# 21K1113/Neural_Image_Compression_V2

Measured on AMD Instinct MI355X. Metric: Mpixels/sec train-step (fwd+bwd) + PSNR, 4K RGB, 1/2/4/8 MI355X, higher is better.
Workload: dtype bf16x2-split operands, f32 accumulate

## Files before the change

neural_image_compression_v2_amd/csrc/fused_train16.hpp:

```cpp
#pragma once
#include "fused_kernel.hpp"


#ifndef NIC_T16_HALF16
#define NIC_T16_HALF16 1
#endif
#ifndef NIC_T16_LOFF
#define NIC_T16_LOFF 26
#endif
#ifndef NIC_T16_PIN
#define NIC_T16_PIN 0
#endif
namespace nic {

struct Lds16 {
    static constexpr int LD1 = 80, LD2 = 80, LD3 = 80;
    static constexpr int LDZ = 72, LDX = 88;
    static constexpr int KP = 80;
    static constexpr int OFF_W1 = 0;
    static constexpr int W1LO = kH * LD1;
    static constexpr int OFF_W2 = OFF_W1 + 2 * kH * LD1;
    static constexpr int W2LO = kH * LD2;
    static constexpr int OFF_W3 = OFF_W2 + 2 * kH * LD2;
    static constexpr int W3LO = 4 * LD3;
    static constexpr int OFF_B = OFF_W3 + 2 * 4 * LD3;
    static constexpr int OFF_IMG = OFF_B + 144;
    static constexpr int DZLO = 16 * LDZ, OFF_A1 = 2 * 16 * LDZ, OFF_X = 4 * 16 * LDZ, XLO = 16 * LDX, OFF_D3 = OFF_X + 2 * 16 * LDX;
    static constexpr int SPW = OFF_D3 + 128;
    static constexpr int TOTAL = OFF_IMG + 8 * SPW;
    static_assert(TOTAL * 2 <= 163840, "LDS");
    static_assert(OFF_IMG % 8 == 0 && SPW % 8 == 0 && OFF_B % 8 == 0, "16-byte alignment");
    static constexpr int REC_W2 = 0, REC_W1 = 8 * 1024, REC_TAIL = 16 * 1024, REC_WAVE = REC_TAIL + 8 * 256, REC = REC_WAVE + 8 * 320;
};

__host__ __device__ constexpr int slot16_channel(int s, int g) {
    if (s < 12) return 12 * g + s;
    if (s < 15) return 48 + 3 * g + (s - 12);
    if (s == 15) return kSlotZero;
    if (s < 19) return 60 + 3 * g + (s - 16);
    if (s == 19) return g == 0 ? 72 : (g == 1 ? kSlotOne : kSlotZero);
    return kSlotZero;
}
__host__ __device__ constexpr int channel_of_rho16(int rho) {
    if (rho < 64) return slot16_channel(8 * (rho >> 5) + (rho & 7), (rho >> 3) & 3);
    return slot16_channel(16 + (rho & 3), (rho - 64) >> 2);
}
__host__ __device__ constexpr int rho16_of_channel(int ch) {
    for (int rho = 0; rho < Lds16::KP; ++rho)
        if (channel_of_rho16(rho) == ch) return rho;
    return -1;
}
__host__ __device__ constexpr int pos16(int h) { return 32 * (h >> 5) + 8 * ((h >> 2) & 3) + 4 * ((h >> 4) & 1) + (h & 3); }
__host__ __device__ constexpr int hid16(int pos) { return 16 * (2 * (pos >> 5) + ((pos >> 2) & 1)) + 4 * ((pos >> 3) & 3) + (pos & 3); }

typedef __attribute__((address_space(3))) const u32x4 lds_cu4;
typedef __attribute__((address_space(3))) u32x4 lds_u4;
__device__ __forceinline__ bf16x8 ld_frag(lds_cbf* p) { return __builtin_bit_cast(bf16x8, *reinterpret_cast<lds_cu4*>(p)); }
__device__ __forceinline__ void st_frag(lds_bf* p, const bf16x8& f) { *reinterpret_cast<lds_u4*>(p) = __builtin_bit_cast(u32x4, f); }
__device__ __forceinline__ bf16x8 half_frag(s16x4 a) {
    const s16x8 v = {a[0], a[1], a[2], a[3], 0, 0, 0, 0};
    return __builtin_bit_cast(bf16x8, v);
}
struct Half2 {
    s16x4 hi, lo;
};
__device__ __forceinline__ f32x4 mfma16h_bf(s16x4 a, s16x4 b, f32x4 c) { return __builtin_amdgcn_mfma_f32_16x16x16bf16_1k(a, b, c, 0, 0, 0); }
__device__ __forceinline__ f32x4 mfma16h_split(const Half2& a, const Half2& b, f32x4 c) {
    c = mfma16h_bf(a.lo, b.hi, c);
    c = mfma16h_bf(a.hi, b.lo, c);
    return mfma16h_bf(a.hi, b.hi, c);
}
__device__ __forceinline__ f32x4 mfma16_split(const Frag2& a, const Frag2& b, f32x4 c) {
    c = mfma16_bf(a.lo, b.hi, c);
    c = mfma16_bf(a.hi, b.lo, c);
    return mfma16_bf(a.hi, b.hi, c);
}
__device__ __forceinline__ Frag2 split_pair(const f32x4& a, const f32x4& b) {
    const float x[8] = {a[0], a[1], a[2], a[3], b[0], b[1], b[2], b[3]};
    return split8(x);
}
__device__ __forceinline__ lds_bf* opaque(lds_bf* p) {
#ifndef NIC_NO_OPAQUE_PTR
    asm volatile("" : "+v"(p));
#endif
    return p;
}

#ifndef NIC_T16_PF
#define NIC_T16_PF 2
#endif
template <int NT, bool ZERO = false, class LoadA>
__device__ __forceinline__ void kstep16(f32x4 (&acc)[NT], const Frag2& bf, LoadA&& load_a) {
    constexpr int PF = NIC_T16_PF < NT ? NIC_T16_PF : NT;
    Frag2 af[PF];
#pragma unroll
    for (int t = 0; t < PF; ++t) af[t] = load_a(t);
#pragma unroll
    for (int t = 0; t < NT; ++t) {
        acc[t] = mfma16_split(af[t % PF], bf, ZERO ? f32x4(0.f) : acc[t]);
        if (t + PF < NT) af[t % PF] = load_a(t + PF);
    }
}

struct CellRaw16 {
    float g0[kC];
    float g1[4 * 3];
};
struct GridAcc16 {
    float g1[4 * 3];
};

__device__ __forceinline__ int opaque_i(int v) {
#ifndef NIC_NO_OPAQUE_LANE
    asm volatile("" : "+v"(v));
#endif
    return v;
}

__device__ __forceinline__ float grid_load16(const char* base, uint32_t ob, int kind, const FusedParams& p) {
    if (kind == 0) return *reinterpret_cast<const float*>(base + ob);
    if (kind == 3) {
        const float n = (float)*reinterpret_cast<const uint8_t*>(base + ob) - p.dq_sub;
        const float q = mul_rn(n, p.dq_rcp);
        return fmaf(fmaf(-q, p.dq_den, n), p.dq_rcp, q);
    }
    const uint32_t hbits = *reinterpret_cast<const uint16_t*>(base + ob);
    if (kind == 1) return __builtin_bit_cast(float, hbits << 16);
    return (float)__builtin_bit_cast(_Float16, (uint16_t)hbits);
}
__device__ __forceinline__ void gather_cell16_kind(const FusedParams& p, const int kind, uint32_t off0, uint32_t off1, int g, CellRaw16& raw) {
    const uint32_t eb = kind == 0 ? 4u : (kind == 3 ? 1u : 2u);
    const uint32_t pb0 = (uint32_t)p.g0.plane * eb, pb1 = (uint32_t)p.g1.plane * eb;
    {
        uint32_t ob = (off0 + (uint32_t)p.g0.at(g >> 1, g & 1, 0)) * eb;
        const char* base = reinterpret_cast<const char*>(p.g0.p);
#pragma unroll
        for (int c = 0; c < kC; ++c, ob += pb0) raw.g0[c] = grid_load16(base, ob, kind, p);
    }
#pragma unroll
    for (int c4 = 0; c4 < 4; ++c4) {
        uint32_t ob = (off1 + (uint32_t)p.g1.at(c4 >> 1, c4 & 1, 0)) * eb + (uint32_t)(3 * g) * pb1;
        const char* base = reinterpret_cast<const char*>(p.g1.p);
#pragma unroll
        for (int cc = 0; cc < 3; ++cc, ob += pb1) raw.g1[c4 * 3 + cc] = grid_load16(base, ob, kind, p);
    }
}
__device__ __forceinline__ void gather_cell16(const FusedParams& p, uint32_t off0, uint32_t off1, int g, CellRaw16& raw) {
    gather_cell16_kind(p, p.grid_kind, off0, off1, g, raw);
}
__device__ __forceinline__ void gather_cell16_switched(const FusedParams& p, uint32_t off0, uint32_t off1, int g, CellRaw16& raw) {
    switch (p.grid_kind) {
        case 0: gather_cell16_kind(p, 0, off0, off1, g, raw); break;
        case 1: gather_cell16_kind(p, 1, off0, off1, g, raw); break;
        case 3: gather_cell16_kind(p, 3, off0, off1, g, raw); break;
        default: gather_cell16_kind(p, 2, off0, off1, g, raw); break;
    }
}

template <class L>
__device__ __forceinline__ void encode16(const FusedParams& p, const int (&q)[3], int g, float (&xs)[20], EncCtx& cx, const CellRaw16& raw) {
    const nic_path_desc& d = p.d;
    const int e = d.log2_step;
    const Axis ax = axis_coords(q[0], e), ay = axis_coords(q[1], e);
    cx.kx = ax.k1; cx.ky = ay.k1; cx.kz = 0.f;
#pragma unroll
    for (int c = 0; c < kC; ++c) xs[c] = raw.g0[c];
    {
        const float c = (g >> 1) ? ay.t1 : ax.t1;
#pragma unroll
        for (int i = 0; i < 3; ++i) {
            const int r = 3 * (g & 1) + i;
            float v;
            if (L::PE == NIC_PE_TRIANGULAR) {
                v = tri_pe_row(c, r, kP);
            } else {
                const int k = r >> 1;
                const float dv = k == 0 ? d.pe_div[0] : (k == 1 ? d.pe_div[1] : d.pe_div[2]);
                float sv, cv;
                sincos_cw(mul_rn(c, dv), sv, cv);
                v = (r & 1) ? cv : sv;
            }
            xs[15 + i] = v;
        }
        xs[18] = g == 0 ? d.lod_value : (g == 1 ? 1.0f : 0.f);
    }
    const G1FactorsT<2> gf = g1_factors<2>(d.g1_weight_mode, cx.kx, cx.ky, 0.f);
#pragma unroll
    for (int cc = 0; cc < 3; ++cc) {
        float sum = 0.f;
#pragma unroll
        for (int c4 = 0; c4 < 4; ++c4) {
            const uint32_t b = (gf.bits >> (3 * c4)) & 7u;
            float v = raw.g1[c4 * 3 + cc];
            v = mul_rn(v, (b & 1u) ? gf.fx[1] : gf.fx[0]);
            v = mul_rn(v, (b & 2u) ? gf.fy[1] : gf.fy[0]);
            sum = c4 == 0 ? v : add_rn(sum, v);
        }
        xs[12 + cc] = sum;
    }
}
__host__ __device__ constexpr int xs_of_slot(int s) { return s < 15 ? s : s - 1; }

template <class L>
__device__ __forceinline__ void add_noise16(const NoiseSrc& ns, uint64_t sample_global, int64_t n_local, int g, float (&xs)[20]) {
    if (ns.mode == NIC_NOISE_NONE) return;
    if (ns.mode == NIC_NOISE_TENSOR) {
        const float* row = ns.tensor + n_local * L::CIN;
#pragma unroll
        for (int s = 0; s < 20; ++s) {
            if (s == 15) continue;
            const int ch0 = slot16_channel(s, 0);
            if (s == 19) { xs[18] += g == 0 ? row[72] : 0.f; continue; }
            const int stride = slot16_channel(s, 1) - ch0;
            xs[xs_of_slot(s)] += row[ch0 + stride * g];
        }
        return;
    }
    const U4 b = noise_block(ns, sample_global, g);
#pragma unroll
    for (int f = 0; f < 18; ++f) xs[f] += noise_field(ns, b, f);
    const float nl = noise_field(ns, b, 18);
    xs[18] += g == 0 ? nl : 0.f;
}

__device__ __forceinline__ int shfl_lane(int v, int src_lane) { return __builtin_amdgcn_ds_bpermute(src_lane << 2, v); }
__device__ __forceinline__ float shfl_lane(float v, int src_lane) { return __builtin_bit_cast(float, __builtin_amdgcn_ds_bpermute(src_lane << 2, __builtin_bit_cast(int, v))); }
__device__ __forceinline__ void combine_g1_lanes16(GridAcc16& ga, uint32_t off1, const int (&blk)[3], int lane, int lw) {
    const int T[2] = {1 << lw, 16 >> lw};
    const int STR[2] = {1, 1 << lw};
    const int pl = lane & 15;
    const int lc[2] = {pl & (T[0] - 1), pl >> lw};
#pragma unroll
    for (int a = 0; a < 2; ++a) {
        const bool odd = blk[a] & 1;
        const int pc = lc[a] + (odd ? -1 : 1);
        const bool inb = pc >= 0 && pc < T[a];
        const int partner = inb ? lane + (odd ? -STR[a] : STR[a]) : lane;
        const bool pair = inb && (uint32_t)shfl_lane((int)off1, partner) == off1;
#pragma unroll
        for (int i = 0; i < 12; ++i) {
            const float pv = shfl_lane(ga.g1[i], partner);
            ga.g1[i] = pair ? (odd ? 0.f : ga.g1[i] + pv) : ga.g1[i];
        }
    }
}

__device__ __forceinline__ void preadd_x16(f32x4 (&dxacc)[4], uint32_t off0, int ln) {
    const int n16 = ln & 15, g = ln >> 4;
    const bool recv = g < 2;
    const bool inb = recv ? n16 >= 1 : n16 <= 14;
    const int partner = inb ? (recv ? ln + 31 : ln - 31) : ln;
    const uint32_t poff = (uint32_t)shfl_lane((int)off0, partner);
    const bool pair = inb && (recv ? off0 == poff + 1u : poff == off0 + 1u);
#pragma unroll
    for (int c = 0; c < kC; ++c) {
        const float pv = shfl_lane(dxacc[c >> 2][c & 3], partner);
        dxacc[c >> 2][c & 3] = pair ? (recv ? dxacc[c >> 2][c & 3] + pv : 0.f) : dxacc[c >> 2][c & 3];
    }
}
template <int NW, class Barrier>
__device__ __forceinline__ void preadd_y16(f32x4 (&dxacc)[4], uint32_t off0, uint32_t row, int ln, int wave, lds_f* reg0, int region, Barrier&& barrier) {
    typedef __attribute__((address_space(3))) uint32_t lds_u32_t;
    const int g = ln >> 4;
    lds_f* const mine = opaque(reg0 + wave * region + ln);
    const bool up = (g & 1) != 0;
    ((lds_u32_t*)mine)[12 * 64] = off0;
    if (up) {
#pragma unroll
        for (int i = 0; i < 12; ++i) mine[i * 64] = dxacc[i >> 2][i & 3];
    }
    barrier();
    const int pw = up ? wave + 1 : wave - 1;
    const bool inw = pw >= 0 && pw < NW;
    lds_cf* const theirs = opaque(reg0 + (inw ? pw : wave) * region + (up ? ln - 16 : ln + 16));
    const uint32_t poff = ((const lds_u32_t*)theirs)[12 * 64];
    const bool pair = inw && (up ? poff == off0 + row : off0 == poff + row);
    if (!up) {
#pragma unroll
        for (int i = 0; i < 12; ++i) {
            const float pv = theirs[i * 64];
            dxacc[i >> 2][i & 3] += pair ? pv : 0.f;
        }
    } else {
#pragma unroll
        for (int i = 0; i < 12; ++i) dxacc[i >> 2][i & 3] = pair ? 0.f : dxacc[i >> 2][i & 3];
    }
    barrier();
}

struct Seg16 {
    int tile0, rg, t_end, base0, lstride, n_my, tiles_per_crop, tiles_main, rounds_unit, shift;
};
struct Unit16 {
    int org[3], blk[3];
    int qb[2];
    int lw, crop;
    int base, tile;
    int it_begin, it_len;
    bool tile_ok;
    uint32_t blk_off0, blk_off1;
    CellRaw16 raw;
};
struct UnitFlush16 {
    int blk[3], lw, base, tile;
    bool tile_ok;
    uint32_t blk_off0, blk_off1;
};
template <class L>
__device__ __forceinline__ void unit_header16(const FusedParams& p, const Seg16& sg, int kk, int lane, int wave, Unit16& u) {
    u.base = sg.base0 + (kk < sg.n_my ? kk : 0) * sg.lstride;
    u.tile_ok = u.base + wave < sg.t_end;
    const int unit = u.tile_ok ? u.base + wave : sg.t_end - 1;
    u.tile = sg.tile0 + (unit >> sg.rg);
    u.it_len = sg.rounds_unit;
    u.it_begin = (int)(unit & ((1 << sg.rg) - 1)) * sg.rounds_unit;
    if (sg.shift) {
        if (kk == 0) { u.it_begin += sg.shift; u.it_len -= sg.shift; }
        else if (kk == sg.n_my) u.it_len = sg.shift;
    }
    u.lw = 4;
    u.crop = u.tile / sg.tiles_per_crop;
    const int ln = opaque_i(lane), n16 = ln & 15, g = ln >> 4;
    const int tt = u.tile - u.crop * sg.tiles_per_crop;
    int boff[2];
    if (p.edge_lw < 0 || tt < sg.tiles_main) {
        boff[1] = tt % p.tiles_y;
        boff[0] = (tt / p.tiles_y) * 16;
    } else {
        u.lw = p.edge_lw;
        boff[1] = (tt - sg.tiles_main) * (16 >> u.lw);
        boff[0] = p.full_x * 16;
    }
    const int lc[2] = {n16 & ((1 << u.lw) - 1), n16 >> u.lw};
#pragma unroll
    for (int a = 0; a < 2; ++a) {
        u.org[a] = origin_of(p, u.crop * 2 + a);
        u.blk[a] = (u.org[a] >> p.lm) + boff[a] + lc[a];
    }
    u.org[2] = 0; u.blk[2] = 0;
    u.qb[0] = u.blk[0] << p.lm; u.qb[1] = u.blk[1] << p.lm;
    const int qb[3] = {u.qb[0], u.qb[1], 0};
    cell_offsets<L>(p, qb, u.blk_off0, u.blk_off1);
    gather_cell16_switched(p, u.blk_off0, u.blk_off1, g, u.raw);
}

#ifndef NIC_T16_PREADD
#define NIC_T16_PREADD 2
#endif
#ifndef NIC_T16_LB
#define NIC_T16_LB 512
#endif
constexpr int MODE_TRAIN_RGBX = 4;
template <class L, int MODE>
__global__ void __launch_bounds__(NIC_T16_LB) fused_train16_kernel(FusedParams p) {
    using S = Lds16;
    static_assert(L::DIM == 2 && L::CIN == 73, "the 16-sample training kernel is built for the 2D slot layouts");
    static_assert(MODE != MODE_INFER, "training kernel");
    constexpr int LD1 = S::LD1, LD2 = S::LD2, LD3 = S::LD3, LDZ = S::LDZ, LDX = S::LDX;
    __shared__ __attribute__((aligned(16))) __bf16 smem16[S::TOTAL];
    lds_bf* const sm = (lds_bf*)smem16;

    const int tid = threadIdx.x, lane = tid & 63;
    const int wave = __builtin_amdgcn_readfirstlane(tid >> 6);

    stage_all<kH * LD1, 512>(tid,
        [&](int idx) {
            const int o = idx / LD1, rho = idx - o * LD1;
            const int ch = channel_of_rho16(rho);
            const float* src = ch >= 0 ? &p.W[0][o * L::CIN + ch] : &p.b[0][o];
            const float v = *src;
            return (ch >= 0 || ch == kSlotOne) ? v : 0.f;
        },
        [&](int idx, float v) {
            const __bf16 hi = (__bf16)v;
            sm[S::OFF_W1 + idx] = hi;
            sm[S::OFF_W1 + S::W1LO + idx] = (__bf16)(v - (float)hi);
        });
    stage_all<kH * LD2, 512>(tid,
        [&](int idx) {
            const int o = idx / LD2, ps = idx - o * LD2;
            const float v = p.W[1][o * kH + hid16(ps < kH ? ps : 0)];
            return ps < kH ? v : 0.f;
        },
        [&](int idx, float v) {
            const __bf16 hi = (__bf16)v;
            sm[S::OFF_W2 + idx] = hi;
            sm[S::OFF_W2 + S::W2LO + idx] = (__bf16)(v - (float)hi);
        });
    stage_all<4 * LD3, 512>(tid,
        [&](int idx) {
            const int c = idx / LD3, ps = idx - c * LD3;
            return (c < 3 && ps < kH) ? p.W[2][c * kH + hid16(ps)] : 0.f;
        },
        [&](int idx, float v) {
            const __bf16 hi = (__bf16)v;
            sm[S::OFF_W3 + idx] = hi;
            sm[S::OFF_W3 + S::W3LO + idx] = (__bf16)(v - (float)hi);
        });
    lds_f* const Bs = (lds_f*)(sm + S::OFF_B);
    if (tid < kH) Bs[tid] = p.b[1][tid];
    if (tid >= kH && tid < kH + 4) Bs[tid] = tid - kH < 3 ? p.b[2][tid - kH] : 0.f;
    for (int idx = tid; idx < 8 * S::SPW / 2; idx += 512) ((lds_f*)(sm + S::OFF_IMG))[idx] = 0.f;
    __syncthreads();
    const NoiseSrc nsrc = noise_with_step(p.noise, p.step_dev);

    f32x16 accW2 = f32x16(0.f);
    f32x16 accW1 = f32x16(0.f);
    f32x4 accT = f32x4(0.f);
    f32x4 accW3q = f32x4(0.f), accB2q = f32x4(0.f);
    float accB3[3] = {0.f, 0.f, 0.f}, accLoss = 0.f;
    const int T4 = wave & 3, kh = wave >> 2;
    const int to = T4 >> 1, tk = T4 & 1;
    lds_bf* const img0 = sm + S::OFF_IMG;

#ifdef NIC_STAMPS
    unsigned long long stamp_sum[NIC_NPH];
#pragma unroll
    for (int i = 0; i < NIC_NPH; ++i) stamp_sum[i] = 0;
    unsigned long long stamp_last;
    asm volatile("s_memtime %0\n\ts_waitcnt lgkmcnt(0)" : "=s"(stamp_last)::"memory");
#endif

    constexpr int LOFF = NIC_T16_LOFF;
    int lo_rW = 0, lo_rZ = 0, lo_tW = 0, lo_b44 = 0, lo_tZ = 0, lo_rX = 0;
    {
        const int n16 = lane & 15, g = lane >> 4, q4 = (lane & 15) >> 2, p4 = lane & 3, h32 = lane >> 5, cg = (lane >> 4) & 1;
        if constexpr ((LOFF & 1) != 0) lo_rW = opaque_i(n16 * S::LD1 + 8 * g);
        if constexpr ((LOFF & 2) != 0) lo_rZ = opaque_i(wave * S::SPW + n16 * S::LDZ + 8 * g);
        if constexpr ((LOFF & 4) != 0) lo_tW = opaque_i((4 * g + q4) * S::LD1 + 8 * p4);
        if constexpr ((LOFF & 8) != 0) lo_b44 = opaque_i(wave * S::SPW + 4 * q4 * S::LDZ + 16 * g + 4 * p4);
        if constexpr ((LOFF & 16) != 0) lo_tZ = opaque_i((4 * (wave >> 2)) * S::SPW + (4 * q4 + 2 * h32) * S::LDZ + 16 * cg + 4 * p4);
        if constexpr ((LOFF & 32) != 0) lo_rX = opaque_i(wave * S::SPW + S::OFF_X + n16 * S::LDX + 8 * g);
    }
    const int xcd = blockIdx.x & 7, nb8 = gridDim.x >> 3;
  for (int seg = 0; seg < 2; ++seg) {
    const int seg_tile0 = seg ? (int)p.seg_split : 0;
    const int seg_tiles = seg ? (int)p.n_tiles - (int)p.seg_split : (int)p.seg_split;
    const int rg = seg ? p.rg_log2 : 0;
    if (seg_tiles <= 0) continue;
    const int n_units = seg_tiles << rg;
    const int chunk = (((n_units + 7) >> 3) + 7) & ~7;
    const int t_begin = xcd * chunk;
    const int t_end = t_begin + chunk < n_units ? t_begin + chunk : n_units;
    const int lstride = nb8 * 8;
    const int base0 = t_begin + (int)(blockIdx.x >> 3) * 8;
    const int n_my = base0 < t_end ? (t_end - base0 + lstride - 1) / lstride : 0;
    const int tiles_per_crop = (int)p.tiles_per_crop, tiles_main = (int)p.tiles_main;
    const int rounds_unit = (p.niter * p.passes) >> rg;
    const int nph = rounds_unit >= NIC_PHASES ? NIC_PHASES : (rounds_unit >= 2 ? 2 : 1);
    const int shift = (NIC_STAGGER && (NIC_STAGGER_RG || rg == 0)) ? (int)((blockIdx.x >> 3) & (nph - 1)) * (rounds_unit / nph) : 0;

    const Seg16 sg = {seg_tile0, rg, t_end, base0, lstride, n_my, tiles_per_crop, tiles_main, rounds_unit, shift};
    const int n_pieces = n_my + (shift ? 1 : 0);
    Unit16 u;
    if (n_pieces > 0) unit_header16<L>(p, sg, 0, lane, wave, u);
    STAMP(12);

    for (int kk = 0; kk < n_pieces; ++kk) {
        GridAcc16 gacc;
        f32x4 dxacc[4];
        f32x4 sdz1[4];
        float zero = 0.f;
        asm volatile("" : "+v"(zero));
#pragma unroll
        for (int i = 0; i < 12; ++i) gacc.g1[i] = zero;
#pragma unroll
        for (int t = 0; t < 4; ++t) { dxacc[t] = f32x4(zero); sdz1[t] = f32x4(zero); }

        for (int it = u.it_begin; it < u.it_begin + u.it_len; ++it) {
            f32x4 a1[4], d1[4], a2[4], d2[4];
            float dz3[3];
            float kx1, ky1;
            {
                const int ln = opaque_i(lane), n16 = ln & 15, g = ln >> 4;
                bool valid = u.tile_ok;
                int64_t n;
                int q[3] = {0, 0, 0};
                {
                    const int m1 = (1 << p.lm) - 1;
                    const int pass = it >> (p.lm * 2), its = it & (p.niter - 1);
                    const int j[2] = {its >> p.lm, its & m1};
                    const int ext[2] = {p.d.extent[0], p.d.extent[1]};
                    int idx[2];
#pragma unroll
                    for (int a = 0; a < 2; ++a) {
                        const int i = u.qb[a] + j[a] - u.org[a];
                        valid = valid && i >= 0 && i < ext[a];
                        idx[a] = i < 0 ? 0 : (i >= ext[a] ? ext[a] - 1 : i);
                        q[a] = u.org[a] + idx[a];
                    }
                    n = ((int64_t)u.crop * p.passes + pass) * p.n_per_crop + (int64_t)idx[0] * ext[1] + idx[1];
                }
                float tgt[3] = {0.f, 0.f, 0.f};
                if (MODE == MODE_TRAIN_RGBX) {
                    const uint32_t off = (uint32_t)q[0] * (uint32_t)p.timg_s[0] + (uint32_t)q[1] * (uint32_t)p.timg_s[1];
                    const uint32_t rgbx = reinterpret_cast<const uint32_t*>(p.timg)[off];
#pragma unroll
                    for (int c = 0; c < 3; ++c) {
                        const float u = (float)((rgbx >> (8 * c)) & 255u);
                        const float t0 = mul_rn(u, p.timg_rcp);
                        tgt[c] = fmaf(fmaf(-t0, p.timg_den, u), p.timg_rcp, t0);
                    }
                } else if (MODE == MODE_TRAIN_IMG) {
                    const int64_t off = (int64_t)q[0] * p.timg_s[0] + (int64_t)q[1] * p.timg_s[1];
                    uint32_t rgbx = 0u;
                    if (p.timg_u8 == 2) rgbx = reinterpret_cast<const uint32_t*>(p.timg)[off];
#pragma unroll
                    for (int c = 0; c < 3; ++c) {
                        if (p.timg_u8) {
                            const float u = p.timg_u8 == 2 ? (float)((rgbx >> (8 * c)) & 255u) : (float)(reinterpret_cast<const uint8_t*>(p.timg) + c * p.timg_cs)[off];
                            const float t0 = mul_rn(u, p.timg_rcp);
                            tgt[c] = fmaf(fmaf(-t0, p.timg_den, u), p.timg_rcp, t0);
                        } else {
                            tgt[c] = (reinterpret_cast<const float*>(p.timg) + c * p.timg_cs)[off];
                        }
                    }
                } else {
                    const float* tp = (MODE == MODE_TRAIN_MSE ? p.target : p.dy) + n * 3;
#pragma unroll
                    for (int c = 0; c < 3; ++c) tgt[c] = tp[c];
                }
                float xs[20];
                {
                    EncCtx cx;
                    encode16<L>(p, q, g, xs, cx, u.raw);
                    kx1 = cx.kx; ky1 = cx.ky;
                    add_noise16<L>(nsrc, (uint64_t)(p.d.sample_base + n), n, g, xs);
                }
                if (it == u.it_begin) STAMP(11);
                else STAMP(0);
                lds_bf* const imgw = img0 + wave * S::SPW;
                {
                    lds_cbf* const w_row = opaque((lds_cbf*)(sm + ((LOFF & 1) ? lo_rW : n16 * LD1 + 8 * g)));
                    lds_cbf* const w1_row2 = opaque((lds_cbf*)(sm + S::OFF_W1 + 64 + ((LOFF & 1) ? lo_rW - 4 * g : n16 * LD1 + 4 * g)));
                    lds_bf* const x_st = (LOFF & 32) ? opaque(img0 + lo_rX) : opaque(imgw + S::OFF_X + n16 * LDX + 8 * g);
                    lds_bf* const x_st2 = (LOFF & 32) ? opaque(img0 + 64 + lo_rX - 4 * g) : opaque(imgw + S::OFF_X + n16 * LDX + 64 + 4 * g);
                    f32x4 z[4];
#pragma unroll
                    for (int s = 0; s < 2; ++s) {
                        const float xv[8] = {xs[8 * s], xs[8 * s + 1], xs[8 * s + 2], xs[8 * s + 3], xs[8 * s + 4], xs[8 * s + 5], xs[8 * s + 6],
                                             s == 0 ? xs[7] : 0.f};
                        const Frag2 bf = split8(xv);
                        st_frag(&x_st[32 * s], bf.hi);
                        st_frag(&x_st[S::XLO + 32 * s], bf.lo);
                        auto la = [&](int t) {
                            Frag2 a;
                            a.hi = ld_frag(&w_row[S::OFF_W1 + 16 * t * LD1 + 32 * s]);
                            a.lo = ld_frag(&w_row[S::OFF_W1 + S::W1LO + 16 * t * LD1 + 32 * s]);
                            return a;
                        };
                        if (s == 0) kstep16<4, true>(z, bf, la);
                        else kstep16<4>(z, bf, la);
                    }
                    {
                        const float xv[8] = {xs[15], xs[16], xs[17], xs[18], 0.f, 0.f, 0.f, 0.f};
                        const Frag2 bf = split8(xv);
                        const s16x8 bh = __builtin_bit_cast(s16x8, bf.hi), bl = __builtin_bit_cast(s16x8, bf.lo);
                        *reinterpret_cast<lds_s16x4*>(x_st2) = s16x4{bh[0], bh[1], bh[2], bh[3]};
                        *reinterpret_cast<lds_s16x4*>(x_st2 + S::XLO) = s16x4{bl[0], bl[1], bl[2], bl[3]};
#if NIC_T16_HALF16
                        const Half2 bq = {s16x4{bh[0], bh[1], bh[2], bh[3]}, s16x4{bl[0], bl[1], bl[2], bl[3]}};
#pragma unroll
                        for (int t = 0; t < 4; ++t) {
                            const Half2 a = {*reinterpret_cast<lds_cs16x4*>(&w1_row2[16 * t * LD1]), *reinterpret_cast<lds_cs16x4*>(&w1_row2[S::W1LO + 16 * t * LD1])};
                            z[t] = mfma16h_split(a, bq, z[t]);
                        }
#else
                        kstep16<4>(z, bf, [&](int t) {
                            Frag2 a;
                            a.hi = half_frag(*reinterpret_cast<lds_cs16x4*>(&w1_row2[16 * t * LD1]));
                            a.lo = half_frag(*reinterpret_cast<lds_cs16x4*>(&w1_row2[S::W1LO + 16 * t * LD1]));
                            return a;
                        });
#endif
                    }
#pragma unroll
                    for (int t = 0; t < 4; ++t) gelu_and_grad4(z[t], a1[t], d1[t]);
                    if (NIC_T16_PIN & 1) {
#pragma unroll
                        for (int t = 0; t < 4; ++t) asm volatile("" : "+v"(d1[t]));
                    }
                    lds_cf* const b2_row = opaque(Bs + 4 * g);
                    lds_bf* const a1_st = (LOFF & 2) ? opaque(img0 + S::OFF_A1 + lo_rZ) : opaque(imgw + S::OFF_A1 + n16 * LDZ + 8 * g);
#pragma unroll
                    for (int t = 0; t < 4; ++t) z[t] = ld4(&b2_row[16 * t]);
#pragma unroll
                    for (int s = 0; s < 2; ++s) {
                        const Frag2 bf = split_pair(a1[2 * s], a1[2 * s + 1]);
                        st_frag(&a1_st[32 * s], bf.hi);
                        st_frag(&a1_st[S::DZLO + 32 * s], bf.lo);
                        kstep16<4>(z, bf, [&](int t) {
                            Frag2 a;
                            a.hi = ld_frag(&w_row[S::OFF_W2 + 16 * t * LD2 + 32 * s]);
                            a.lo = ld_frag(&w_row[S::OFF_W2 + S::W2LO + 16 * t * LD2 + 32 * s]);
                            return a;
                        });
                    }
#pragma unroll
                    for (int t = 0; t < 4; ++t) gelu_and_grad4(z[t], a2[t], d2[t]);
                    if ((NIC_T16_PIN & 2) || ((NIC_T16_PIN & 4) && L::PE == NIC_PE_SINUSOIDAL)) {
#pragma unroll
                        for (int t = 0; t < 4; ++t) asm volatile("" : "+v"(d2[t]));
                    }
                }
                float yv[3];
                {
                    lds_cbf* const w3_row = opaque((lds_cbf*)(sm + S::OFF_W3 + (n16 < 3 ? n16 : 3) * LD3 + 8 * g));
                    lds_bf* const dz_st = (LOFF & 2) ? opaque(img0 + lo_rZ) : opaque(imgw + n16 * LDZ + 8 * g);
                    f32x4 z3;
#pragma unroll
                    for (int s = 0; s < 2; ++s) {
                        Frag2 af;
                        af.hi = ld_frag(&w3_row[32 * s]);
                        af.lo = ld_frag(&w3_row[S::W3LO + 32 * s]);
                        const Frag2 bf = split_pair(a2[2 * s], a2[2 * s + 1]);
                        st_frag(&dz_st[32 * s], bf.hi);
                        st_frag(&dz_st[S::DZLO + 32 * s], bf.lo);
                        z3 = mfma16_split(af, bf, s == 0 ? f32x4(0.f) : z3);
                    }
                    lds_cf* const b3_row = opaque(Bs + kH);
#pragma unroll
                    for (int c = 0; c < 3; ++c) yv[c] = sigmoid_f(z3[c] + b3_row[c]);
                }
                STAMP(1);
                const bool own = valid && g == 0;
                if (p.y != nullptr && own) {
#pragma unroll
                    for (int c = 0; c < 3; ++c) p.y[n * 3 + c] = yv[c];
                }
#pragma unroll
                for (int c = 0; c < 3; ++c) {
                    float gr;
                    if (MODE == MODE_TRAIN_MSE || MODE == MODE_TRAIN_IMG || MODE == MODE_TRAIN_RGBX) {
                        const float diff = own ? yv[c] - tgt[c] : 0.f;
                        accLoss += diff * diff;
                        gr = p.grad_scale * diff;
                    } else {
                        gr = own ? tgt[c] : 0.f;
                    }
                    dz3[c] = gr * yv[c] * (1.0f - yv[c]);
                    accB3[c] += dz3[c];
                }
                if (g == 0) {
                    lds_bf* const d3_st = opaque(imgw + S::OFF_D3 + 4 * (n16 & 3) + (n16 >> 2));
#pragma unroll
                    for (int c = 0; c < 3; ++c) {
                        const __bf16 hi = (__bf16)dz3[c];
                        d3_st[c * 16] = hi;
                        d3_st[64 + c * 16] = (__bf16)(dz3[c] - (float)hi);
                    }
                }
            }
            wave_lds_fence();
            f32x4 dz1[4];
            {
                const int ln = opaque_i(lane), n16 = ln & 15, g = ln >> 4, q4 = (ln & 15) >> 2, p4 = ln & 3;
                lds_bf* const imgw = img0 + wave * S::SPW;
                lds_cbf* const dz_b44 = (LOFF & 8) ? opaque((lds_cbf*)(img0 + lo_b44)) : opaque((lds_cbf*)(imgw + 4 * q4 * LDZ + 16 * g + 4 * p4));
                {
                    lds_cbf* const d3_a44 = opaque((lds_cbf*)(imgw + S::OFF_D3 + (ln & 3) * 16));
                    s16x4 bh[4], bl[4], ah[4], al[4];
#pragma unroll
                    for (int r = 0; r < 4; ++r) {
                        bh[r] = tr4(&dz_b44[r * LDZ]);
                        bl[r] = tr4(&dz_b44[S::DZLO + r * LDZ]);
                        ah[r] = *reinterpret_cast<lds_cs16x4*>(&d3_a44[4 * r]);
                        al[r] = *reinterpret_cast<lds_cs16x4*>(&d3_a44[64 + 4 * r]);
                    }
#pragma unroll
                    for (int r = 0; r < 4; ++r) {
                        accW3q = mfma4_bf(al[r], bh[r], accW3q);
                        accW3q = mfma4_bf(ah[r], bl[r], accW3q);
                        accW3q = mfma4_bf(ah[r], bh[r], accW3q);
                    }
                }
                f32x4 dz2[4];
                {
                    lds_cbf* const w3_tr = opaque((lds_cbf*)(sm + S::OFF_W3 + q4 * LD3 + 8 * p4));
                    const float dzv[8] = {dz3[0], dz3[1], dz3[2], 0.f, 0.f, 0.f, 0.f, 0.f};
                    const Frag2 bf = split8(dzv);
                    const s16x8 b3h = __builtin_bit_cast(s16x8, bf.hi), b3l = __builtin_bit_cast(s16x8, bf.lo);
                    const Half2 bq3 = {s16x4{b3h[0], b3h[1], b3h[2], b3h[3]}, s16x4{b3l[0], b3l[1], b3l[2], b3l[3]}};
#pragma unroll
                    for (int t = 0; t < 4; ++t) {
                        const s16x4 ahh = tr4(&w3_tr[32 * (t >> 1) + 4 * (t & 1)]);
                        const s16x4 all = tr4(&w3_tr[S::W3LO + 32 * (t >> 1) + 4 * (t & 1)]);
#if NIC_T16_HALF16
                        const Half2 aq = {ahh, all};
                        dz2[t] = mfma16h_split(aq, bq3, f32x4(0.f)) * d2[t];
#else
                        Frag2 af;
                        af.hi = join8(ahh, ahh);
                        af.lo = join8(all, all);
                        dz2[t] = mfma16_split(af, bf, f32x4(0.f)) * d2[t];
#endif
                    }
                }
                STAMP(2);
                wave_lds_fence();
                {
                    lds_cbf* const w2_tr = opaque((lds_cbf*)(sm + S::OFF_W2 + ((LOFF & 4) ? lo_tW : (4 * g + q4) * LD2 + 8 * p4)));
                    lds_bf* const dz_st = (LOFF & 2) ? opaque(img0 + lo_rZ) : opaque(imgw + n16 * LDZ + 8 * g);
                    f32x4 acc[4];
#pragma unroll
                    for (int s = 0; s < 2; ++s) {
                        const Frag2 bf = split_pair(dz2[2 * s], dz2[2 * s + 1]);
                        st_frag(&dz_st[32 * s], bf.hi);
                        st_frag(&dz_st[S::DZLO + 32 * s], bf.lo);
                        auto la = [&](int t) {
                            const int co = 32 * (t >> 1) + 4 * (t & 1);
                            Frag2 a;
                            a.hi = join8(tr4(&w2_tr[32 * s * LD2 + co]), tr4(&w2_tr[(32 * s + 16) * LD2 + co]));
                            a.lo = join8(tr4(&w2_tr[S::W2LO + 32 * s * LD2 + co]), tr4(&w2_tr[S::W2LO + (32 * s + 16) * LD2 + co]));
                            return a;
                        };
                        if (s == 0) kstep16<4, true>(acc, bf, la);
                        else kstep16<4>(acc, bf, la);
                    }
#pragma unroll
                    for (int t = 0; t < 4; ++t) {
                        dz1[t] = acc[t] * d1[t];
                        sdz1[t] += dz1[t];
                    }
                }
                wave_lds_fence();
                {
                    const s16x4 ones = {0x3F80, 0x3F80, 0x3F80, 0x3F80};
                    s16x4 bh[4], bl[4];
#pragma unroll
                    for (int r = 0; r < 4; ++r) {
                        bl[r] = tr4(&dz_b44[S::DZLO + r * LDZ]);
                        bh[r] = tr4(&dz_b44[r * LDZ]);
                    }
#pragma unroll
                    for (int r = 0; r < 4; ++r) {
                        accB2q = mfma4_bf(ones, bl[r], accB2q);
                        accB2q = mfma4_bf(ones, bh[r], accB2q);
                    }
                }
            }
            STAMP(3);
            wg_lds_barrier();
            STAMP(4);
            {
                const int ln = opaque_i(lane), q4 = (ln & 15) >> 2, p4 = ln & 3, h32 = ln >> 5, cg = (ln >> 4) & 1;
                lds_cbf* const dz_t32 = opaque((lds_cbf*)(img0 + 32 * to + ((LOFF & 16) ? lo_tZ : (4 * kh) * S::SPW + (4 * q4 + 2 * h32) * LDZ + 16 * cg + 4 * p4)));
                lds_cbf* const a1_t32 = opaque((lds_cbf*)(img0 + S::OFF_A1 + 32 * tk + ((LOFF & 16) ? lo_tZ : (4 * kh) * S::SPW + (4 * q4 + 2 * h32) * LDZ + 16 * cg + 4 * p4)));
#pragma unroll
                for (int v = 0; v < 4; ++v) {
                    Frag2 af, bf;
                    af.hi = join8(tr4(&dz_t32[v * S::SPW]), tr4(&dz_t32[v * S::SPW + LDZ]));
                    bf.lo = join8(tr4(&a1_t32[v * S::SPW + S::DZLO]), tr4(&a1_t32[v * S::SPW + S::DZLO + LDZ]));
                    af.lo = join8(tr4(&dz_t32[v * S::SPW + S::DZLO]), tr4(&dz_t32[v * S::SPW + S::DZLO + LDZ]));
                    bf.hi = join8(tr4(&a1_t32[v * S::SPW]), tr4(&a1_t32[v * S::SPW + LDZ]));
                    accW2 = mfma_split(af, bf, accW2);
                }
            }
            STAMP(5);
            wg_lds_barrier();
            STAMP(6);
            {
                const int ln = opaque_i(lane), n16 = ln & 15, g = ln >> 4, q4 = (ln & 15) >> 2, p4 = ln & 3;
                lds_cbf* const w1_tr = opaque((lds_cbf*)(sm + S::OFF_W1 + ((LOFF & 4) ? lo_tW : (4 * g + q4) * LD1 + 8 * p4)));
                lds_bf* const dz_st = (LOFF & 2) ? opaque(img0 + lo_rZ) : opaque(img0 + wave * S::SPW + n16 * LDZ + 8 * g);
                f32x4 dx3[1];
#pragma unroll
                for (int s = 0; s < 2; ++s) {
                    const Frag2 bf = split_pair(dz1[2 * s], dz1[2 * s + 1]);
                    st_frag(&dz_st[32 * s], bf.hi);
                    st_frag(&dz_st[S::DZLO + 32 * s], bf.lo);
                    auto la = [&](int) {
                        constexpr int co = 32 * (3 >> 1) + 4 * (3 & 1);
                        Frag2 a;
                        a.hi = join8(tr4(&w1_tr[32 * s * LD1 + co]), tr4(&w1_tr[(32 * s + 16) * LD1 + co]));
                        a.lo = join8(tr4(&w1_tr[S::W1LO + 32 * s * LD1 + co]), tr4(&w1_tr[S::W1LO + (32 * s + 16) * LD1 + co]));
                        return a;
                    };
                    if (s == 0) kstep16<1, true>(dx3, bf, la);
                    else kstep16<1>(dx3, bf, la);
                }
                const G1FactorsT<2> gf = g1_factors<2>(p.d.g1_weight_mode, kx1, ky1, 0.f);
#pragma unroll
                for (int c4 = 0; c4 < 4; ++c4) {
                    const float w = g1_corner_factor<2>(gf, c4);
#pragma unroll
                    for (int cc = 0; cc < 3; ++cc) gacc.g1[c4 * 3 + cc] = fmaf(dx3[0][cc], w, gacc.g1[c4 * 3 + cc]);
                }
            }
            STAMP(7);
            wg_lds_barrier();
            STAMP(8);
            {
                const int ln = opaque_i(lane), g = ln >> 4, q4 = (ln & 15) >> 2, p4 = ln & 3, h32 = ln >> 5, cg = (ln >> 4) & 1;
                lds_cbf* const dz_t32 = opaque((lds_cbf*)(img0 + 32 * to + ((LOFF & 16) ? lo_tZ : (4 * kh) * S::SPW + (4 * q4 + 2 * h32) * LDZ + 16 * cg + 4 * p4)));
                lds_cbf* const x_t32 = opaque((lds_cbf*)(img0 + (4 * kh) * S::SPW + S::OFF_X + (4 * q4 + 2 * h32) * LDX + 32 * tk + 16 * cg + 4 * p4));
#pragma unroll
                for (int v = 0; v < 4; ++v) {
                    Frag2 af, bf;
                    af.hi = join8(tr4(&dz_t32[v * S::SPW]), tr4(&dz_t32[v * S::SPW + LDZ]));
                    bf.lo = join8(tr4(&x_t32[v * S::SPW + S::XLO]), tr4(&x_t32[v * S::SPW + S::XLO + LDX]));
                    af.lo = join8(tr4(&dz_t32[v * S::SPW + S::DZLO]), tr4(&dz_t32[v * S::SPW + S::DZLO + LDZ]));
                    bf.hi = join8(tr4(&x_t32[v * S::SPW]), tr4(&x_t32[v * S::SPW + LDX]));
                    accW1 = mfma_split(af, bf, accW1);
                }
                lds_cbf* const dz_t16 = opaque((lds_cbf*)(img0 + (4 * kh + (g >> 1)) * S::SPW + (4 * q4 + 2 * (g & 1)) * LDZ + 16 * T4 + 4 * p4));
                lds_cbf* const x_t16 = opaque((lds_cbf*)(img0 + (4 * kh + (g >> 1)) * S::SPW + S::OFF_X + (4 * q4 + 2 * (g & 1)) * LDX + 64 + 4 * p4));
#pragma unroll
                for (int uu = 0; uu < 2; ++uu) {
                    Frag2 af, bf;
                    af.hi = join8(tr4(&dz_t16[2 * uu * S::SPW]), tr4(&dz_t16[2 * uu * S::SPW + LDZ]));
                    af.lo = join8(tr4(&dz_t16[2 * uu * S::SPW + S::DZLO]), tr4(&dz_t16[2 * uu * S::SPW + S::DZLO + LDZ]));
                    bf.hi = join8(tr4(&x_t16[2 * uu * S::SPW]), tr4(&x_t16[2 * uu * S::SPW + LDX]));
                    bf.lo = join8(tr4(&x_t16[2 * uu * S::SPW + S::XLO]), tr4(&x_t16[2 * uu * S::SPW + S::XLO + LDX]));
                    accT = mfma16_split(af, bf, accT);
                }
            }
            STAMP(9);
            wg_lds_barrier();
            STAMP(10);
        }

        UnitFlush16 fu = {{u.blk[0], u.blk[1], 0}, u.lw, u.base, u.tile, u.tile_ok, u.blk_off0, u.blk_off1};
        asm volatile("" : "+v"(fu.blk_off0), "+v"(fu.blk_off1), "+v"(fu.blk[0]), "+v"(fu.blk[1]));
        if (kk + 1 < n_pieces) unit_header16<L>(p, sg, kk + 1, lane, wave, u);
        STAMP(12);

        {
            const int ln = opaque_i(lane), g = ln >> 4, q4 = (ln & 15) >> 2, p4 = ln & 3;
            lds_cbf* const w1_tr = opaque((lds_cbf*)(sm + S::OFF_W1 + ((LOFF & 4) ? lo_tW : (4 * g + q4) * LD1 + 8 * p4)));
#pragma unroll
            for (int s = 0; s < 2; ++s) {
                const float x[8] = {sdz1[2 * s][0], sdz1[2 * s][1], sdz1[2 * s][2], sdz1[2 * s][3],
                                    sdz1[2 * s + 1][0], sdz1[2 * s + 1][1], sdz1[2 * s + 1][2], sdz1[2 * s + 1][3]};
                const Frag2 bf = split8(x);
                float r[8];
#pragma unroll
                for (int i = 0; i < 8; ++i) r[i] = (x[i] - (float)bf.hi[i]) - (float)bf.lo[i];
                const bf16x8 b3 = split8(r).hi;
#pragma unroll
                for (int t = 0; t < 3; ++t) {
                    const int co = 32 * (t >> 1) + 4 * (t & 1);
                    Frag2 a;
                    a.hi = join8(tr4(&w1_tr[32 * s * LD1 + co]), tr4(&w1_tr[(32 * s + 16) * LD1 + co]));
                    a.lo = join8(tr4(&w1_tr[S::W1LO + 32 * s * LD1 + co]), tr4(&w1_tr[S::W1LO + (32 * s + 16) * LD1 + co]));
                    f32x4 c = mfma16_bf(a.lo, bf.lo, s == 0 ? f32x4(0.f) : dxacc[t]);
                    c = mfma16_bf(a.hi, b3, c);
                    dxacc[t] = mfma16_split(a, bf, c);
                }
            }
        }
        {
            const int ln = opaque_i(lane), g = ln >> 4;
            combine_g1_lanes16(gacc, fu.blk_off1, fu.blk, ln, fu.lw);
            bool flush = true;
            if (NIC_GROUP_SUM && rg > 0) {
                lds_f* const reg0 = (lds_f*)img0;
                constexpr int REGION = S::SPW / 2;
                static_assert(24 * 64 <= REGION, "group-sum scratch");
                int leader = wave;
                if (fu.tile_ok)
                    for (int w = wave - 1; w >= 4 * kh; --w)
                        if (seg_tile0 + ((fu.base + w) >> rg) == fu.tile) leader = w;
                if (leader != wave) {
                    lds_f* const mine = opaque(reg0 + wave * REGION + ln);
#pragma unroll
                    for (int i = 0; i < 12; ++i) mine[i * 64] = dxacc[i >> 2][i & 3];
#pragma unroll
                    for (int i = 0; i < 12; ++i) mine[(12 + i) * 64] = gacc.g1[i];
                }
                wg_lds_barrier();
                if (leader == wave && fu.tile_ok) {
                    for (int w = wave + 1; w < 4 * kh + 4; ++w) {
                        if (fu.base + w >= t_end || seg_tile0 + ((fu.base + w) >> rg) != fu.tile) break;
                        lds_cf* const theirs = opaque(reg0 + w * REGION + ln);
#pragma unroll
                        for (int i = 0; i < 12; ++i) dxacc[i >> 2][i & 3] += theirs[i * 64];
#pragma unroll
                        for (int i = 0; i < 12; ++i) gacc.g1[i] += theirs[(12 + i) * 64];
                    }
                }
                wg_lds_barrier();
                flush = leader == wave;
            }
            if (flush && NIC_T16_PREADD) preadd_x16(dxacc, fu.blk_off0, ln);
            if (NIC_T16_PREADD >= 2 && rg == 0 && (p.preadd_y || !NIC_PREADD_Y_SMALL)) {
                static_assert(13 * 64 <= S::SPW / 2, "pre-add scratch");
                preadd_y16<8>(dxacc, fu.blk_off0, (uint32_t)p.g0.nx, ln, wave, (lds_f*)img0, S::SPW / 2, [&]() { wg_lds_barrier(); });
            }
            if (flush) {
                const uint32_t pb0 = (uint32_t)p.g0.plane * 4u, pb1 = (uint32_t)p.g1.plane * 4u;
                uint32_t nz0 = 0u, nz1 = 0u;
#pragma unroll
                for (int c = 0; c < kC; ++c) {
                    nz0 |= __builtin_bit_cast(uint32_t, dxacc[c >> 2][c & 3]);
                    nz1 |= __builtin_bit_cast(uint32_t, gacc.g1[c]);
                }
                if ((nz0 << 1) != 0u) {
                    uint32_t ob = (fu.blk_off0 + (uint32_t)p.g0.at(g >> 1, g & 1, 0)) * 4u;
                    char* gbase = reinterpret_cast<char*>(p.g0_grad);
#pragma unroll
                    for (int c = 0; c < kC; ++c, ob += pb0) atomicAdd(reinterpret_cast<float*>(gbase + ob), dxacc[c >> 2][c & 3]);
                }
                if ((nz1 << 1) != 0u) {
#pragma unroll
                    for (int c4 = 0; c4 < 4; ++c4) {
                        uint32_t ob = (fu.blk_off1 + (uint32_t)p.g1.at(c4 >> 1, c4 & 1, 0)) * 4u + (uint32_t)(3 * g) * pb1;
                        char* gbase = reinterpret_cast<char*>(p.g1_grad);
#pragma unroll
                        for (int cc = 0; cc < 3; ++cc, ob += pb1) atomicAdd(reinterpret_cast<float*>(gbase + ob), gacc.g1[c4 * 3 + cc]);
                    }
                }
            }
        }
        STAMP(13);
    }
  }
#ifdef NIC_STAMPS
    if (lane == 0) {
        unsigned long long* dst = reinterpret_cast<unsigned long long*>(p.partials + (size_t)gridDim.x * S::REC) + ((size_t)blockIdx.x * 8 + wave) * 16;
#pragma unroll
        for (int i = 0; i < NIC_NPH; ++i) dst[i] = stamp_sum[i];
    }
#endif

    float* rec = p.partials + (int64_t)blockIdx.x * S::REC;
#pragma unroll
    for (int r = 0; r < 16; ++r) {
        rec[S::REC_W2 + wave * 1024 + r * 64 + lane] = accW2[r];
        rec[S::REC_W1 + wave * 1024 + r * 64 + lane] = accW1[r];
    }
#pragma unroll
    for (int r = 0; r < 4; ++r) rec[S::REC_TAIL + wave * 256 + r * 64 + lane] = accT[r];
    float* tail = rec + S::REC_WAVE + wave * 320;
    tail[lane] = accB2q[0];
#pragma unroll
    for (int c = 0; c < 3; ++c) tail[64 + 64 * c + lane] = accW3q[c];
#pragma unroll
    for (int c = 0; c < 4; ++c) {
        float v = c < 3 ? accB3[c] : accLoss;
#pragma unroll
        for (int m = 32; m > 0; m >>= 1) v += __shfl_xor(v, m);
        if (lane == 0) tail[256 + c] = v;
    }
}

constexpr int kR16_SRC = 4096 + 4096 + 1024 + 320;
#ifndef NIC_R16_SLICES
#define NIC_R16_SLICES 8
#endif
template <class L>
__global__ void __launch_bounds__(256) reduce16_kernel(const float* partials, int n_rec, nic_mlp_grads gr, float* loss, float loss_scale, const StepTail tl) {
    if (tail_block(tl)) return;
    using S = Lds16;
    constexpr int SL = NIC_R16_SLICES, OUTS = 256 / SL;
    __shared__ float red[SL][OUTS];
    const int slice = threadIdx.x / OUTS, oi = threadIdx.x % OUTS;
    const int gid = blockIdx.x * OUTS + oi;
    const bool live = gid < kR16_SRC;
    int nsrc = 0, off0 = 0, stride = 0;
    float* dst = nullptr;
    bool is_loss = false;
    if (live) {
        if (gid < 8192) {
            const int u = gid & 4095, T4 = u >> 10, r = (u >> 6) & 15, l = u & 63;
            const int po = 32 * (T4 >> 1) + (r & 3) + 8 * (r >> 2) + 4 * (l >> 5), col = 32 * (T4 & 1) + (l & 31);
            const int o = hid16(po);
            nsrc = 2; stride = 4 * 1024;
            if (gid < 4096) {
                off0 = S::REC_W1 + u;
                const int ch = channel_of_rho16(col);
                if (ch >= 0) dst = gr.w[0] ? gr.w[0] + o * L::CIN + ch : nullptr;
                else if (ch == kSlotOne) dst = gr.b[0] ? gr.b[0] + o : nullptr;
            } else {
                off0 = S::REC_W2 + u;
                dst = gr.w[1] ? gr.w[1] + o * kH + hid16(col) : nullptr;
            }
        } else if (gid < 9216) {
            const int u = gid - 8192, wq = u >> 8, r = (u >> 6) & 3, l = u & 63;
            const int o = hid16(16 * wq + r + 4 * (l >> 4)), ch = channel_of_rho16(64 + (l & 15));
            off0 = S::REC_TAIL + u; nsrc = 2; stride = 4 * 256;
            if (ch >= 0) dst = gr.w[0] ? gr.w[0] + o * L::CIN + ch : nullptr;
            else if (ch == kSlotOne) dst = gr.b[0] ? gr.b[0] + o : nullptr;
        } else {
            const int u = gid - 9216;
            off0 = S::REC_WAVE + u; nsrc = 8; stride = 320;
            if (u < 64) dst = gr.b[1] ? gr.b[1] + hid16(u) : nullptr;
            else if (u < 256) dst = gr.w[2] ? gr.w[2] + ((u - 64) >> 6) * kH + hid16(u & 63) : nullptr;
            else if (u < 259) dst = gr.b[2] ? gr.b[2] + (u - 256) : nullptr;
            else if (u == 259) { dst = loss; is_loss = true; }
        }
    }
    float part[8] = {0.f, 0.f, 0.f, 0.f, 0.f, 0.f, 0.f, 0.f};
    const int per = (n_rec + SL - 1) / SL;
    const int w_lo = slice * per, w_hi = (w_lo + per < n_rec) ? w_lo + per : n_rec;
    if (live && dst != nullptr) {
        for (int k = 0; k < nsrc; ++k) {
            const float* src = partials + off0 + k * stride;
            int w = w_lo;
            for (; w + 8 <= w_hi; w += 8) {
#pragma unroll
                for (int j = 0; j < 8; ++j) part[j] += src[(int64_t)(w + j) * S::REC];
            }
            for (; w < w_hi; ++w) part[0] += src[(int64_t)w * S::REC];
        }
    }
    red[slice][oi] = ((part[0] + part[1]) + (part[2] + part[3])) + ((part[4] + part[5]) + (part[6] + part[7]));
    __syncthreads();
    if (slice != 0 || !live || dst == nullptr) return;
    float acc = red[0][oi];
#pragma unroll
    for (int sl = 1; sl < SL; ++sl) acc += red[sl][oi];
    if (is_loss) *dst = acc * loss_scale;
    else tail_store(tl, dst, acc);
}

}
```

Measured before the change: 4129.

## Shadow dz1 split and dX kstep under W2 MFMA phase with sched group barriers

Moves the split of dz1 and the dX kstep (W1 transpose reads plus MFMAs) out of their own barrier-delimited phase into the W2 gradient MFMA loop. The stage between two barriers is reduced to just the LDS stores. The g1 corner-factor accumulation is deferred into the W1 gradient loop. Sched_group_barrier hints interleave MFMA, VALU and LDS reads so the extra work hides under MFMA latency. This raises register pressure by keeping zf/dx3 live across barriers, and the fixed scheduling masks may not match the real instruction mix.

```diff
diff --git a/neural_image_compression_v2_amd/csrc/fused_train16.hpp b/neural_image_compression_v2_amd/csrc/fused_train16.hpp
--- a/neural_image_compression_v2_amd/csrc/fused_train16.hpp
+++ b/neural_image_compression_v2_amd/csrc/fused_train16.hpp
@@ -7,6 +7,9 @@
 #endif
 #ifndef NIC_T16_LOFF
 #define NIC_T16_LOFF 26
+#endif
+#ifndef NIC_T16_SHADOW_SGB
+#define NIC_T16_SHADOW_SGB 1
 #endif
 #ifndef NIC_T16_PIN
 #define NIC_T16_PIN 0
@@ -742,10 +745,14 @@
             STAMP(3);
             wg_lds_barrier();
             STAMP(4);
+            Frag2 zf[2];
+            f32x4 dx3[1];
+            lds_bf* dz1_st;
             {
-                const int ln = opaque_i(lane), q4 = (ln & 15) >> 2, p4 = ln & 3, h32 = ln >> 5, cg = (ln >> 4) & 1;
+                const int ln = opaque_i(lane), g = ln >> 4, q4 = (ln & 15) >> 2, p4 = ln & 3, h32 = ln >> 5, cg = (ln >> 4) & 1;
                 lds_cbf* const dz_t32 = opaque((lds_cbf*)(img0 + 32 * to + ((LOFF & 16) ? lo_tZ : (4 * kh) * S::SPW + (4 * q4 + 2 * h32) * LDZ + 16 * cg + 4 * p4)));
                 lds_cbf* const a1_t32 = opaque((lds_cbf*)(img0 + S::OFF_A1 + 32 * tk + ((LOFF & 16) ? lo_tZ : (4 * kh) * S::SPW + (4 * q4 + 2 * h32) * LDZ + 16 * cg + 4 * p4)));
+                lds_cbf* const w1_tr = opaque((lds_cbf*)(sm + S::OFF_W1 + ((LOFF & 4) ? lo_tW : (4 * g + q4) * LD1 + 8 * p4)));
 #pragma unroll
                 for (int v = 0; v < 4; ++v) {
                     Frag2 af, bf;
@@ -754,38 +761,42 @@
                     af.lo = join8(tr4(&dz_t32[v * S::SPW + S::DZLO]), tr4(&dz_t32[v * S::SPW + S::DZLO + LDZ]));
                     bf.hi = join8(tr4(&a1_t32[v * S::SPW]), tr4(&a1_t32[v * S::SPW + LDZ]));
                     accW2 = mfma_split(af, bf, accW2);
-                }
+                    if (v < 2) {
+                        zf[v] = split_pair(dz1[2 * v], dz1[2 * v + 1]);
+                    } else {
+                        const int s = v - 2;
+                        auto la = [&](int) {
+                            constexpr int co = 32 * (3 >> 1) + 4 * (3 & 1);
+                            Frag2 a;
+                            a.hi = join8(tr4(&w1_tr[32 * s * LD1 + co]), tr4(&w1_tr[(32 * s + 16) * LD1 + co]));
+                            a.lo = join8(tr4(&w1_tr[S::W1LO + 32 * s * LD1 + co]), tr4(&w1_tr[S::W1LO + (32 * s + 16) * LD1 + co]));
+                            return a;
+                        };
+                        if (s == 0) kstep16<1, true>(dx3, zf[s], la);
+                        else kstep16<1>(dx3, zf[s], la);
+                    }
+                }
+#if NIC_T16_SHADOW_SGB
+                __builtin_amdgcn_sched_group_barrier(0x100, 8, 0);
+#pragma unroll
+                for (int i = 0; i < 18; ++i) {
+                    __builtin_amdgcn_sched_group_barrier(0x008, 1, 0);
+                    __builtin_amdgcn_sched_group_barrier(0x002, 4, 0);
+                    __builtin_amdgcn_sched_group_barrier(0x100, 2, 0);
+                }
+#endif
+#pragma unroll
+                for (int s = 0; s < 2; ++s) asm volatile("" : "+v"(zf[s].hi), "+v"(zf[s].lo));
+                asm volatile("" : "+v"(dx3[0]));
+                dz1_st = (LOFF & 2) ? opaque(img0 + lo_rZ) : opaque(img0 + wave * S::SPW + (ln & 15) * LDZ + 8 * g);
             }
             STAMP(5);
             wg_lds_barrier();
             STAMP(6);
-            {
-                const int ln = opaque_i(lane), n16 = ln & 15, g = ln >> 4, q4 = (ln & 15) >> 2, p4 = ln & 3;
-                lds_cbf* const w1_tr = opaque((lds_cbf*)(sm + S::OFF_W1 + ((LOFF & 4) ? lo_tW : (4 * g + q4) * LD1 + 8 * p4)));
-                lds_bf* const dz_st = (LOFF & 2) ? opaque(img0 + lo_rZ) : opaque(img0 + wave * S::SPW + n16 * LDZ + 8 * g);
-                f32x4 dx3[1];
-#pragma unroll
-                for (int s = 0; s < 2; ++s) {
-                    const Frag2 bf = split_pair(dz1[2 * s], dz1[2 * s + 1]);
-                    st_frag(&dz_st[32 * s], bf.hi);
-                    st_frag(&dz_st[S::DZLO + 32 * s], bf.lo);
-                    auto la = [&](int) {
-                        constexpr int co = 32 * (3 >> 1) + 4 * (3 & 1);
-                        Frag2 a;
-                        a.hi = join8(tr4(&w1_tr[32 * s * LD1 + co]), tr4(&w1_tr[(32 * s + 16) * LD1 + co]));
-                        a.lo = join8(tr4(&w1_tr[S::W1LO + 32 * s * LD1 + co]), tr4(&w1_tr[S::W1LO + (32 * s + 16) * LD1 + co]));
-                        return a;
-                    };
-                    if (s == 0) kstep16<1, true>(dx3, bf, la);
-                    else kstep16<1>(dx3, bf, la);
-                }
-                const G1FactorsT<2> gf = g1_factors<2>(p.d.g1_weight_mode, kx1, ky1, 0.f);
-#pragma unroll
-                for (int c4 = 0; c4 < 4; ++c4) {
-                    const float w = g1_corner_factor<2>(gf, c4);
-#pragma unroll
-                    for (int cc = 0; cc < 3; ++cc) gacc.g1[c4 * 3 + cc] = fmaf(dx3[0][cc], w, gacc.g1[c4 * 3 + cc]);
-                }
+#pragma unroll
+            for (int s = 0; s < 2; ++s) {
+                st_frag(&dz1_st[32 * s], zf[s].hi);
+                st_frag(&dz1_st[S::DZLO + 32 * s], zf[s].lo);
             }
             STAMP(7);
             wg_lds_barrier();
@@ -794,6 +805,7 @@
                 const int ln = opaque_i(lane), g = ln >> 4, q4 = (ln & 15) >> 2, p4 = ln & 3, h32 = ln >> 5, cg = (ln >> 4) & 1;
                 lds_cbf* const dz_t32 = opaque((lds_cbf*)(img0 + 32 * to + ((LOFF & 16) ? lo_tZ : (4 * kh) * S::SPW + (4 * q4 + 2 * h32) * LDZ + 16 * cg + 4 * p4)));
                 lds_cbf* const x_t32 = opaque((lds_cbf*)(img0 + (4 * kh) * S::SPW + S::OFF_X + (4 * q4 + 2 * h32) * LDX + 32 * tk + 16 * cg + 4 * p4));
+                asm volatile("" : "+v"(dx3[0]), "+v"(kx1), "+v"(ky1));
 #pragma unroll
                 for (int v = 0; v < 4; ++v) {
                     Frag2 af, bf;
@@ -802,6 +814,15 @@
                     af.lo = join8(tr4(&dz_t32[v * S::SPW + S::DZLO]), tr4(&dz_t32[v * S::SPW + S::DZLO + LDZ]));
                     bf.hi = join8(tr4(&x_t32[v * S::SPW]), tr4(&x_t32[v * S::SPW + LDX]));
                     accW1 = mfma_split(af, bf, accW1);
+                    if (v == 0) {
+                        const G1FactorsT<2> gf = g1_factors<2>(p.d.g1_weight_mode, kx1, ky1, 0.f);
+#pragma unroll
+                        for (int c4 = 0; c4 < 4; ++c4) {
+                            const float w = g1_corner_factor<2>(gf, c4);
+#pragma unroll
+                            for (int cc = 0; cc < 3; ++cc) gacc.g1[c4 * 3 + cc] = fmaf(dx3[0][cc], w, gacc.g1[c4 * 3 + cc]);
+                        }
+                    }
                 }
                 lds_cbf* const dz_t16 = opaque((lds_cbf*)(img0 + (4 * kh + (g >> 1)) * S::SPW + (4 * q4 + 2 * (g & 1)) * LDZ + 16 * T4 + 4 * p4));
                 lds_cbf* const x_t16 = opaque((lds_cbf*)(img0 + (4 * kh + (g >> 1)) * S::SPW + S::OFF_X + (4 * q4 + 2 * (g & 1)) * LDX + 64 + 4 * p4));
@@ -814,6 +835,15 @@
                     bf.lo = join8(tr4(&x_t16[2 * uu * S::SPW + S::XLO]), tr4(&x_t16[2 * uu * S::SPW + S::XLO + LDX]));
                     accT = mfma16_split(af, bf, accT);
                 }
+#if NIC_T16_SHADOW_SGB
+                __builtin_amdgcn_sched_group_barrier(0x100, 8, 0);
+#pragma unroll
+                for (int i = 0; i < 18; ++i) {
+                    __builtin_amdgcn_sched_group_barrier(0x008, 1, 0);
+                    __builtin_amdgcn_sched_group_barrier(0x002, 3, 0);
+                    __builtin_amdgcn_sched_group_barrier(0x100, 3, 0);
+                }
+#endif
             }
             STAMP(9);
             wg_lds_barrier();
```

Result: slower. 3963 (-4.0%).
